# lhwright13/Hybrid-Classical-and-Reinforcement-Learning-Aircraft-Controllers

Hardware: AMD Instinct MI355X
Metric: env-steps/sec (whole node), rate-control task, batch 65536 per GPU (higher is better)
Workload: dtype f32 compute / f64 state

## Files before the change

### hybrid-classical-and-reinforcement-learning-aircraft-controllers_amd/_lib.py

```python
import ctypes as C
import os

_HERE = os.path.dirname(os.path.abspath(__file__))
LIB_PATH = os.environ.get("FDYN_LIB", os.path.join(_HERE, "csrc", "libfdyn_hip.so"))

FDYN_OK, FDYN_ERR_BAD_DT, FDYN_ERR_BAD_TYPES, FDYN_ERR_BAD_SIZE, FDYN_ERR_NULL = 0, -1, -2, -3, -4

_p = C.c_void_p
_i, _i64, _u64, _d, _f = C.c_int, C.c_int64, C.c_uint64, C.c_double, C.c_float

_SIXDOF = [_p, _p, _p, _p, _i, _i64, _d, _i, _p, _p]
_CASCADE = [_p, _p, _p, _p, _p, _i, _p, _p, _p, _i, _i64, _d, _i, _p, _p, _p]
_AGENT = [_i, _p, _p, _p, _p, _i, _p, _i, _p, _p, _i64, _d, _i, _p, _p]
_HYBRID = [_i, _p, _p, _p, _p, _p, _i, _p, _p, _p, _p, _i, _p, _p, _i, _p, _p, _p, _p, _p, _i64, _d, _p]
_ENV_RESET = [_p, _p, _p, _p, _p, _p, _p, _i, _u64, _p, _i64, _p]
_ENV_STEP = [_p, _p, _p, _p, _p, _i, _p, _p, _p, _p, _p, _p, _p, _p, _i, _u64, _i, _f, _p, _p, _p, _p, _p, _p, _p, _p, _p,
             _i, _i64, _p]
_ENV_RESET_DR = _ENV_RESET[:-1] + [_p, _p, _p]
_ENV_STEP_DR = _ENV_STEP[:-1] + [_p, _p, _p]

SIGNATURES = {
    "fdyn_abi_version": (_i, []),
    "fdyn_num_substeps": (_i, [_d, _d]),
    "fdyn_device_info": (_i, [C.POINTER(_i), C.POINTER(_i), C.c_char_p, _i]),
    "fdyn_event_capacity": (_i64, [_i64]),
    "fdyn_sixdof_step_f64": (_i, _SIXDOF), "fdyn_sixdof_step_mixed": (_i, _SIXDOF), "fdyn_sixdof_step_f32": (_i, _SIXDOF),
    "fdyn_derived_f64": (_i, [_p, _i64, _p, _p]), "fdyn_derived_f32": (_i, [_p, _i64, _p, _p]),
    "fdyn_pid_compute_batch": (_i, [_p, _i, _p, _p, _p, _f, _p, _i64, _p]),
    "fdyn_cascade_step_f64": (_i, _CASCADE), "fdyn_cascade_step_mixed": (_i, _CASCADE), "fdyn_cascade_step_f32": (_i, _CASCADE),
    "fdyn_rate_env_reset_f64": (_i, _ENV_RESET), "fdyn_rate_env_reset_mixed": (_i, _ENV_RESET),
    "fdyn_rate_env_reset_f32": (_i, _ENV_RESET),
    "fdyn_rate_env_step_f64": (_i, _ENV_STEP), "fdyn_rate_env_step_mixed": (_i, _ENV_STEP),
    "fdyn_rate_env_step_f32": (_i, _ENV_STEP),
    "fdyn_rate_env_reset_dr_f64": (_i, _ENV_RESET_DR), "fdyn_rate_env_reset_dr_mixed": (_i, _ENV_RESET_DR),
    "fdyn_rate_env_reset_dr_f32": (_i, _ENV_RESET_DR),
    "fdyn_rate_env_step_dr_f64": (_i, _ENV_STEP_DR), "fdyn_rate_env_step_dr_mixed": (_i, _ENV_STEP_DR),
    "fdyn_rate_env_step_dr_f32": (_i, _ENV_STEP_DR),
    "fdyn_lstm_cell_fwd": (_i, [_p, _i, _p, _p, _p, _p, _p, _i64, _i, _p]),
    "fdyn_lstm_cell_bwd": (_i, [_p, _i, _p, _p, _p, _p, _p, _p, _i64, _i, _p]),
    "fdyn_lstm_seq_fwd": (_i, [_p, _i, _p, _p, _p, _p, _p, _p, _i64, _p, _p, _i64, _i64, _i, _p]),
    "fdyn_lstm_seq_bwd": (_i, [_p, _i, _p, _p, _p, _p, _p, _i64, _p, _p, _p, _p, _i64, _i, _p]),
    "fdyn_lstm_seq_bwd_bsum": (_i, [_p, _i, _p, _p, _p, _p, _p, _i64, _p, _p, _p, _p, _p, _i64, _i64, _i, _p]),
    "fdyn_lstm_seq_bwd_pre": (_i, [_p, _i, _p, _i64, _p, _p, _p, _p, _p, _i64, _p, _p, _p, _p, _p, _i64, _i64, _i, _p]),
    "fdyn_lstm_cell0_fwd": (_i, [_p, _i, _p, _p, _i64, _i, _p]),
    "fdyn_lstm_cell0_bwd": (_i, [_p, _i, _p, _p, _p, _i64, _i64, _i, _p]),
    "fdyn_colsum_partials": (_i, [_p, _i64, _i, _p, _p, _p]),
    "fdyn_episode_flags": (_i, [_p, _p, _p, _p, _p, _i64, _p]),
    "fdyn_policy_trunks": (_i, [_p, _p, _p, _p, _p, _p, _p, _p, _i64, _p]),
    "fdyn_policy_trunks_heads": (_i, [_p] * 11 + [_u64, _p, _i, _p, _p, _p, _i64, _p]),
    "fdyn_agent_step_f64": (_i, _AGENT), "fdyn_agent_step_mixed": (_i, _AGENT), "fdyn_agent_step_f32": (_i, _AGENT),
    "fdyn_hybrid_step_f64": (_i, _HYBRID), "fdyn_hybrid_step_mixed": (_i, _HYBRID), "fdyn_hybrid_step_f32": (_i, _HYBRID),
    "fdyn_colsum_ws_floats": (_i64, [_i64, _i, _i64, _i]),
# ... 91 lines not shown
```

### hybrid-classical-and-reinforcement-learning-aircraft-controllers_amd/csrc/fdyn_kernels.hip

```cpp
#include <hip/hip_runtime.h>
#include <stdint.h>
#include <math.h>
#include <string.h>
#include <stdlib.h>
#include "fdyn_core.hpp"
#include "../../include/fdyn.h"

using namespace fdyn;

#define FD_BLOCK 256
#define FD_MAX_TYPES 8
#define FD_WAVE 64

template <typename T>
__device__ __forceinline__ void stage(T* dst, const T* __restrict__ src, int n)
{
    for (int i = threadIdx.x; i < n; i += blockDim.x) dst[i] = src[i];
}

template <bool FAST>
__device__ __forceinline__ void stage_params(double* s_params, const double* __restrict__ params, int n_types)
{
    for (int i = threadIdx.x; i < n_types * FD_NP_USED; i += blockDim.x) {
        const int t = i / FD_NP_USED, k = i - t * FD_NP_USED;
// ... 19 lines not shown
    w.d = int(threadIdx.x) < n_types * NDL ? params[t * FD_NP + Params<double>::derive_source(threadIdx.x - t * NDL)] : 1.0;
    return w;
}
template <bool FAST>
__device__ __forceinline__ void stage_params_finish(double* s_params, const StagedParamWords& w, int n_types)
{
    const int i0 = threadIdx.x, i1 = FD_BLOCK + threadIdx.x;
    const int t0 = i0 / FD_NP_USED, t1 = i1 / FD_NP_USED;
    if (i0 < n_types * FD_NP_USED) s_params[t0 * FD_NP_STAGED + (i0 - t0 * FD_NP_USED)] = w.v0;
    if (i1 < n_types * FD_NP_USED) s_params[t1 * FD_NP_STAGED + (i1 - t1 * FD_NP_USED)] = w.v1;
    constexpr int NDL = Params<double>::FD_ND_LANES;
    if (int(threadIdx.x) < n_types * NDL) {
        const int t = threadIdx.x / NDL;
        Params<double>::derive_lane_from<FAST>(threadIdx.x - t * NDL, w.d, s_params + t * FD_NP_STAGED);
    }
}

template <typename G>
__device__ __forceinline__ void stage_cascade_consts(G* s_consts, const double* __restrict__ consts)
{
    for (int k = threadIdx.x; k < FD_NC; k += blockDim.x) s_consts[k] = G(consts[k]);
    if (threadIdx.x < 2) {
        const double bank = consts[threadIdx.x == 0 ? FD_C_WP_MAX_BANK_RAD : FD_C_LOS_MAX_BANK_RAD];
        s_consts[FD_CD_WP_INV_G_TAN_BANK + threadIdx.x] = G(1.0 / (9.81 * ::tan(bank)));
    }
}

struct LaneMap { int64_t i, wave_first; int lane; bool on; };
__device__ __forceinline__ LaneMap lane_map(int64_t n)
{
// ... 537 lines not shown
    x[6] = rec[FD_R_ROLL]; x[7] = rec[FD_R_PITCH]; x[8] = rec[FD_R_YAW];
    x[9] = rec[FD_R_P]; x[10] = rec[FD_R_Q]; x[11] = rec[FD_R_R];
#pragma unroll
    for (int k = 0; k < 3; ++k) { e.cmd[k] = E(0); e.prev_err[k] = E(0); e.sign_changes[k] = E(0); e.prev_action[k] = E(0); }
#pragma unroll
    for (int k = 0; k < 4; ++k) e.sched[k] = E(0);
    e.prev_action[3] = E(0.5);
    if (cmd_type == FD_CMD_STEP) {
        e.cmd[0] = E(rec[FD_R_CMD0]); e.cmd[1] = E(rec[FD_R_CMD1]); e.cmd[2] = E(rec[FD_R_CMD2]);
    } else if (cmd_type == FD_CMD_RAMP || cmd_type == FD_CMD_SINE) {
        e.sched[0] = E(rec[FD_R_CMD0]); e.sched[1] = E(rec[FD_R_CMD1]); e.sched[2] = E(rec[FD_R_CMD2]); e.sched[3] = E(rec[FD_R_CMD3]);
    }
    e.settle_timer = E(0); e.is_settled = E(0); e.time = E(0); e.ep_return = E(0);
}

template <typename G>
__device__ __forceinline__ void load_env_consts(const double* __restrict__ EC, EnvConsts<G>& ec)
{
    ec.dt = G(EC[FD_EC_DT]);
    ec.max_steps = int(EC[FD_EC_MAX_STEPS]);
    ec.cmd_type = int(EC[FD_EC_CMD_TYPE]);
    ec.scale = G(EC[FD_EC_DIFFICULTY_SCALE]);
    ec.mr0 = G(EC[FD_EC_MAX_RATE_P]); ec.mr1 = G(EC[FD_EC_MAX_RATE_Q]); ec.mr2 = G(EC[FD_EC_MAX_RATE_R]);
    const double r = EC[FD_EC_DT] / EC[FD_EC_DT_PHYSICS];
    const long ns = long(r);
    ec.n_sub = ns < 1 ? 1 : int(ns);
    const double dts = EC[FD_EC_DT];
    int k = 0;
    if (dts >= 1.0e-3) { double t = 0.0; while (t < 0.2 && k < 256) { t += dts; ++k; } }
    else k = int(0.2 / dts) + 1;
    ec.settle_steps = k;
}

template <typename G>
__device__ __forceinline__ void fetch_reset_record(const double* __restrict__ pool, int pool_depth, uint64_t seed,
                                                   int64_t i, int32_t episode, const EnvConsts<G>& ec, G (&rec)[FD_NR])
{
    if (pool) {
        const double* r = pool + (i * pool_depth + (episode % pool_depth)) * FD_NR;
#pragma unroll
        for (int k = 0; k < FD_NR; ++k) rec[k] = G(r[k]);
    } else {
        device_reset_record<G>(seed, uint32_t(i), uint32_t(episode), ec, rec);
    }
}

__device__ __forceinline__ void store_obs_tile(float* tile , const float (&o)[FD_OBS_DIM], int lane,
                                               float* __restrict__ obs_out, int64_t wave_first, int64_t n)
{
    int64_t valid = n - wave_first;
    valid = valid < 0 ? 0 : (valid < FD_WAVE ? valid : FD_WAVE);
    float* dst = obs_out + wave_first * FD_OBS_DIM;
    static_assert(FD_OBS_DIM == 18 && FD_WAVE == 64, "the full-wave path below moves 64 x 18 floats as 288 float4");
    if (valid == FD_WAVE && (reinterpret_cast<uintptr_t>(dst) & 15) == 0) {
        float2* row = reinterpret_cast<float2*>(tile + lane * FD_OBS_DIM);
#pragma unroll
// ... 152 lines not shown
extern "C" int fdyn_debug_read_counts(unsigned* out, int count, int clear)
{
    int rc = int(hipMemcpyFromSymbol(out, HIP_SYMBOL(fdyn_dbg_cnt), sizeof(unsigned) * size_t(count)));
    if (clear && rc == 0) {
        void* p = nullptr;
        rc = int(hipGetSymbolAddress(&p, HIP_SYMBOL(fdyn_dbg_cnt)));
        if (rc == 0) rc = int(hipMemset(p, 0, sizeof(unsigned) * 4096 * 8));
    }
    return rc;
}
#else
#define FD_STAMP(K)
#define FD_STAMP_REAL(K)
#endif

template <typename S, typename T, bool OCC2, typename... DRA>
__global__ void __launch_bounds__(FD_BLOCK, OCC2 ? 2 : 1)
rate_env_step_kernel(S* __restrict__ xs, typename EnvOf<S, T>::type* __restrict__ es, int32_t* __restrict__ eis,
                     const uint8_t* __restrict__ type, const double* __restrict__ params, int n_types,
                     const double* __restrict__ EC,
                     const float* __restrict__ actions ,
                     float* __restrict__ pid_state , const float* __restrict__ pid_cfg ,
                     const double* __restrict__ casc_consts , float* __restrict__ actions_out,
                     const S* __restrict__ rw_delta ,
                     const double* __restrict__ pool, int pool_depth, uint64_t seed, int auto_reset, float residual_scale,
                     float* __restrict__ obs_out , float* __restrict__ reward_f32, S* __restrict__ reward_full,
                     uint8_t* __restrict__ terminated, uint8_t* __restrict__ truncated,
                     int32_t* __restrict__ ev_count, int32_t* __restrict__ ev_count_next, int32_t* __restrict__ ev_int,
                     float* __restrict__ ev_flt, int ev_cap, int64_t n, DRA... dra)
{
    constexpr bool DR = sizeof...(DRA) != 0;
    S* dr = nullptr;
    const double* drc = nullptr;
    if constexpr (DR) dr_unpack(dr, drc, dra...);
    __shared__ double s_params[FD_MAX_TYPES * FD_NP_STAGED];
    __shared__ __attribute__((aligned(16))) float s_tile[FD_BLOCK / FD_WAVE][FD_WAVE * (FD_OBS_DIM + 1)];
    __shared__ float s_pid_cfg[3 * FD_NPC];
    __shared__ S s_consts[FD_NC];
    FD_STAMP(0)
    FD_STAMP_REAL(7)
    const LaneMap lm = lane_map(n);
    const int64_t i = lm.i;
    const int lane = lm.lane, wave = threadIdx.x / FD_WAVE;
    const bool active = lm.on;
    EnvConsts<S> ec;
    load_env_consts<S>(EC, ec);
    const bool uses_sched = ec.cmd_type == FD_CMD_RAMP || ec.cmd_type == FD_CMD_SINE;
    const bool residual_mode = actions != nullptr && residual_scale > 0.0f && pid_state != nullptr;
    const bool pid_mode = actions == nullptr || residual_mode;

    using E = typename EnvOf<S, T>::type;
    S x[FD_NX];
    EnvState<E> e;
    int32_t step = 0, episode = 0;
    int ty = 0;
    float4 av = make_float4(0.0f, 0.0f, 0.0f, 0.0f);
    S rec_pre[FD_NR];
    S wair[3] = { S(0), S(0), S(0) }, dsc[5] = { S(1), S(1), S(1), S(1), S(1) };
    const bool pre_drawn = !OCC2 && pool == nullptr && auto_reset != 0;
    constexpr bool EARLY_PARAMS = sizeof(T) == 4;
    StagedParamWords spw = { 0.0, 0.0, 1.0 };
    if constexpr (EARLY_PARAMS) spw = stage_params_early(params, n_types);
    if (active) {
        episode = eis[FD_EI_EPISODE * n + i];
#pragma unroll
        for (int k = 3; k < FD_NX; ++k) x[k] = xs[k * n + i];
        if (actions) av = reinterpret_cast<const float4*>(actions)[i];
        ty = lane_type(type, i, n_types);
#pragma unroll
        for (int k = 0; k < 3; ++k) x[k] = xs[k * n + i];
        step = eis[FD_EI_STEP * n + i];
        env_load<E>(e, es, n, i, uses_sched);
        if (pre_drawn) device_reset_record<S>(seed, uint32_t(i), uint32_t(episode), ec, rec_pre);
        if constexpr (DR) {
#pragma unroll
            for (int k = 0; k < 3; ++k) wair[k] = dr[(FD_DR_WIND_N + k) * n + i] + dr[(FD_DR_GUST_N + k) * n + i];
#pragma unroll
            for (int k = 0; k < 5; ++k) dsc[k] = dr[(FD_DR_MASS_S + k) * n + i];
        }
    }
    if constexpr (EARLY_PARAMS) stage_params_finish<true>(s_params, spw, n_types);
    else stage_params<false>(s_params, params, n_types);
    if (pid_mode) {
        stage(s_pid_cfg, pid_cfg, 3 * FD_NPC);
        for (int k = threadIdx.x; k < FD_NC; k += blockDim.x) s_consts[k] = S(casc_consts[k]);
    }
    __syncthreads();

    if (ev_count_next && blockIdx.x == 0 && threadIdx.x < FD_EV_SHARDS) ev_count_next[threadIdx.x] = 0;

    float o[FD_OBS_DIM];
#pragma unroll
    for (int k = 0; k < FD_OBS_DIM; ++k) o[k] = 0.0f;
    bool done = false, term = false;
    S reward = S(0);

// ... 119 lines not shown
        if (reward_f32) reward_f32[i] = float(reward);
        if (reward_full) reward_full[i] = reward;
        terminated[i] = term ? 1 : 0;
        truncated[i] = trunc ? 1 : 0;
    }

    FD_STAMP(3)
    const unsigned long long done_mask = __ballot(done);
    const bool compact = done_mask != 0ull && ev_count != nullptr;
    int base = 0, prefix = 0;
    const int shard = int(blockIdx.x) & (FD_EV_SHARDS - 1), cap_s = ev_cap / FD_EV_SHARDS;
    if (compact) {
        const int n_done = __popcll(done_mask);
        prefix = __builtin_amdgcn_mbcnt_hi(uint32_t(done_mask >> 32), __builtin_amdgcn_mbcnt_lo(uint32_t(done_mask), 0u));
        const int leader = __ffsll((long long)done_mask) - 1;
        if (lane == leader) base = atomicAdd(ev_count + shard, n_done);
    }
    float o_term[FD_OBS_DIM];
#pragma unroll
    for (int k = 0; k < FD_OBS_DIM; ++k) o_term[k] = o[k];
    const float ret_term = done ? float(e.ep_return) : 0.0f;
    const int32_t len_term = step;

    if (active) {
        if (done && auto_reset) {
            S rec[FD_NR];
            if (pre_drawn) {
#pragma unroll
                for (int k = 0; k < FD_NR; ++k) rec[k] = rec_pre[k];
            } else {
                fetch_reset_record<S>(pool, pool_depth, seed, i, episode, ec, rec);
// ... 5 lines not shown
            using A0 = typename GlueOf<S, T>::type;
            A0 xa[FD_NX];
#pragma unroll
            for (int k = 0; k < FD_NX; ++k) xa[k] = A0(x[k]);
            A0 airspeed, altitude;
            airspeed_altitude<A0>(xa, airspeed, altitude);
            if constexpr (DR) airspeed = air_speed<A0, S>(x, wair);
            env_observation<S, A0, E>(x, e, airspeed, altitude, o);
            if (pid_mode) for (int k = 0; k < 3 * FD_NPS; ++k) pid_state[k * n + i] = 0.0f;
        }
#pragma unroll
        for (int k = 0; k < FD_NX; ++k) xs[k * n + i] = x[k];
        env_store<E>(e, es, n, i, uses_sched);
        eis[FD_EI_STEP * n + i] = step;
        eis[FD_EI_EPISODE * n + i] = episode;
    }
    if (compact) {
        const int leader = __ffsll((long long)done_mask) - 1;
        base = __shfl(base, leader, FD_WAVE);
        const int local = base + prefix;
        if (done && local < cap_s) {
            const int slot = shard * cap_s + local;
            ev_int[slot * FD_EV_NI + FD_EV_ENV] = int32_t(i);
            ev_int[slot * FD_EV_NI + FD_EV_LENGTH] = len_term;
            ev_int[slot * FD_EV_NI + FD_EV_TERMINATED] = term ? 1 : 0;
            ev_flt[slot * FD_EV_NF] = ret_term;
#pragma unroll
            for (int k = 0; k < FD_OBS_DIM; ++k) ev_flt[slot * FD_EV_NF + 1 + k] = o_term[k];
        }
    }
    FD_STAMP(4)
    store_obs_tile(s_tile[wave], o, lane, obs_out, lm.wave_first, n);
    FD_STAMP(5)
#ifdef FD_PHASE_STAMPS
    asm volatile("s_waitcnt vmcnt(0)" ::: "memory");
#endif
    FD_STAMP_REAL(6)
}

static int g_simds = 0;
static int simd_count()
{
    if (!g_simds) {
        int dev = 0; hipDeviceProp_t p;
        g_simds = (hipGetDevice(&dev) == hipSuccess && hipGetDeviceProperties(&p, dev) == hipSuccess) ? p.multiProcessorCount * 4 : 1024;
    }
    return g_simds;
}

template <typename K, typename... A>
static int launch(K kernel, int64_t n, void* stream, A... args)
{
// ... 20 lines not shown
    int32_t* ev_count_next, int32_t* ev_int, float* ev_flt, int ev_cap, int64_t n
#define FD_ENV_STEP_ARGS                                                                                     \
    x, e, ei, type, params, n_types, env_consts, actions, pid_state, pid_cfg, casc_consts, actions_out, rw_delta, pool, \
    pool_depth, seed, auto_reset, residual_scale, obs_out, reward_f32, reward_full, terminated, truncated, ev_count, \
    ev_count_next, ev_int, ev_flt, ev_cap, n

template <typename S, typename E, typename... DRA>
static int env_reset(FD_ENV_RESET_PARAMS(S, E), void* stream, DRA... dra)
{
    if ((... || !dra)) return FDYN_ERR_NULL;
    FD_CHECK_COMMON(n, 1)
    if (pool && pool_depth < 1) return FDYN_ERR_BAD_SIZE;
    return launch(rate_env_reset_kernel<S, E, DRA...>, n, stream, FD_ENV_RESET_ARGS, dra...);
}

template <typename S, typename E, typename T, typename... DRA>
static int env_step(FD_ENV_STEP_PARAMS(S, E), void* stream, DRA... dra)
{
    if ((... || !dra)) return FDYN_ERR_NULL;
    FD_CHECK_COMMON(n, n_types)
    if (pool && pool_depth < 1) return FDYN_ERR_BAD_SIZE;
    if ((!actions || residual_scale > 0.0f) && !(pid_state && pid_cfg && casc_consts)) return FDYN_ERR_NULL;
    if (!obs_out || !terminated || !truncated || !env_consts) return FDYN_ERR_NULL;
    if (ev_count && (!ev_int || !ev_flt)) return FDYN_ERR_NULL;
    if (ev_count && (ev_cap < FD_EV_SHARDS || ev_cap % FD_EV_SHARDS != 0)) return FDYN_ERR_BAD_SIZE;
    constexpr bool FP32 = sizeof(T) == 4;
    const bool occ2 = FP32 && n > int64_t(simd_count()) * FD_WAVE;
    return launch(occ2 ? rate_env_step_kernel<S, T, FP32, DRA...> : rate_env_step_kernel<S, T, false, DRA...>, n, stream,
                  FD_ENV_STEP_ARGS, dra...);
}

extern "C" {

int fdyn_abi_version(void) { return FDYN_ABI_VERSION; }

int fdyn_num_substeps(double dt, double dt_physics)
{
    const double r = dt / dt_physics;
    const long n = long(r);
    return n < 1 ? 1 : int(n);
}

int64_t fdyn_event_capacity(int64_t n)
// ... 94 lines not shown
                      consts, cmd, wps, n_wp, actions, learned, throttle_src, prev_action, obs_out, rate_cmd_out, surf_out, \
                      reached_total, n, S(dt));                                                              \
    }
FD_DEFINE_HYBRID(fdyn_hybrid_step_f64, double, double)
FD_DEFINE_HYBRID(fdyn_hybrid_step_mixed, double, float)
FD_DEFINE_HYBRID(fdyn_hybrid_step_f32, float, float)

FD_DEFINE_CASCADE(fdyn_cascade_step_f64, double, double)
FD_DEFINE_CASCADE(fdyn_cascade_step_mixed, double, float)
FD_DEFINE_CASCADE(fdyn_cascade_step_f32, float, float)

#define FD_DEFINE_ENV(SUFFIX, S, E, T)                                                                       \
    int fdyn_rate_env_reset_##SUFFIX(FD_ENV_RESET_PARAMS(S, E), void* stream)                                \
    { return env_reset<S, E>(FD_ENV_RESET_ARGS, stream); }                                                   \
    int fdyn_rate_env_step_##SUFFIX(FD_ENV_STEP_PARAMS(S, E), void* stream)                                  \
    { return env_step<S, E, T>(FD_ENV_STEP_ARGS, stream); }
FD_DEFINE_ENV(f64, double, double, double)
FD_DEFINE_ENV(mixed, double, float, float)
FD_DEFINE_ENV(f32, float, float, float)

#define FD_DEFINE_ENV_DR(SUFFIX, S, E, T)                                                                    \
    int fdyn_rate_env_reset_dr_##SUFFIX(FD_ENV_RESET_PARAMS(S, E), S* dr, const double* dr_consts, void* stream) \
    { return env_reset<S, E>(FD_ENV_RESET_ARGS, stream, dr, dr_consts); }                                    \
    int fdyn_rate_env_step_dr_##SUFFIX(FD_ENV_STEP_PARAMS(S, E), S* dr, const double* dr_consts, void* stream) \
    { return env_step<S, E, T>(FD_ENV_STEP_ARGS, stream, dr, dr_consts); }
FD_DEFINE_ENV_DR(f64, double, double, double)
FD_DEFINE_ENV_DR(mixed, double, float, float)
FD_DEFINE_ENV_DR(f32, float, float, float)

}
```

### hybrid-classical-and-reinforcement-learning-aircraft-controllers_amd/rate_env.py

```python
from typing import Optional, Sequence

import numpy as np
import torch

from . import _lib, layout as L
from .config import cascade_consts, pid_table
from .params import param_table
from .samplers import COMMAND_TYPE, EpisodeStreams, env_consts, presample_reset_pool


class GpuRateVecEnv:
    def __init__(self, num_envs: int, difficulty: str = "medium", episode_length: float = 10.0, dt: float = 0.02,
                 command_type: str = "step", seed: Optional[int] = None, precision: str = "mixed",
                 sampling: str = "device", pool_depth: int = 8, types: Sequence = ("rc_plane",),
                 type_index: Optional[np.ndarray] = None, event_capacity: Optional[int] = None,
                 numpy_io: bool = False, device=None, residual_scale: float = 0.0, sensor_noise: Optional[dict] = None,
                 disturbances=None):
        self.lib = _lib.load()
        self.device = device or _lib.require_gpu()
        self.num_envs = self.n = int(num_envs)
        self.precision, self.dtype = precision, _lib.state_dtype(precision)
        self.difficulty, self.episode_length, self.dt, self.command_type = difficulty, episode_length, dt, command_type
        self.seed_value = 0 if seed is None else int(seed)
        self.numpy_io = numpy_io
# ... 31 lines not shown
        self.pool, self.pool_depth, self._streams = None, 0, None
        if sampling == "parity":
            seeds = [None if seed is None else seed + i for i in range(n)]
            self.pool_depth = int(pool_depth)
            self.pool = torch.as_tensor(presample_reset_pool(seeds, pool_depth, difficulty, command_type), device=dev)
            if command_type == "random":
                self._streams = [EpisodeStreams(difficulty, command_type, s) for s in seeds]
        elif sampling != "device":
            raise ValueError("sampling must be 'parity' or 'device'")
        self.sensor = None
        if sensor_noise is not None:
            from .sensors import ObservationNoise
            self.sensor = ObservationNoise(sensor_noise, n, dev)
            self._done_mask = torch.zeros(n, dtype=torch.uint8, device=dev)
        self._reset_fn = getattr(self.lib, f"fdyn_rate_env_reset_{precision}")
        self._step_fn = getattr(self.lib, f"fdyn_rate_env_step_{precision}")
        self._pending = None
        self.dr, self.dr_consts, self.disturbances = None, None, None
        if disturbances is not None:
            self.set_disturbances(disturbances)

    def set_disturbances(self, d):
        from .disturbances import Disturbances, as_disturbances, neutral_rows
        d = as_disturbances(d)
        if d is None:
            d = Disturbances()
        self.disturbances = d
        blk = torch.as_tensor(d.block(), device=self.device)
        if self.dr_consts is None:
            self.dr_consts = blk
            self.dr = torch.as_tensor(neutral_rows(self.n), device=self.device).to(self.dtype).contiguous()
            self._reset_fn = getattr(self.lib, f"fdyn_rate_env_reset_dr_{self.precision}")
            self._step_fn = getattr(self.lib, f"fdyn_rate_env_step_dr_{self.precision}")
        else:
            self.dr_consts.copy_(blk)
        return d

    def _dr_args(self):
        return () if self.dr is None else (_lib.ptr(self.dr), _lib.ptr(self.dr_consts))

    def reset(self, mask: Optional[torch.Tensor] = None):
        m = None if mask is None else mask.to(torch.uint8).contiguous()
        rc = self._reset_fn(_lib.ptr(self.x), _lib.ptr(self.e), _lib.ptr(self.ei), _lib.ptr(self.pid_state),
                            _lib.ptr(m), _lib.ptr(self.env_consts), _lib.ptr(self.pool), self.pool_depth,
                            self.seed_value, _lib.ptr(self.obs), self.n, *self._dr_args(), _lib.current_stream())
        _lib.check(rc, "RateControlEnv.reset")
        if self.sensor is not None:
            if m is None:
                self.sensor.reset()
                self.sensor.apply(self.obs)
            else:
                keep, keep_bias, mb = self.obs.clone(), self.sensor.gyro_bias.clone(), m.bool()
                self.sensor.apply(self.obs, m)
                self.obs.copy_(torch.where(mb[:, None], self.obs, keep))
                self.sensor.gyro_bias.copy_(torch.where(mb[None, :], self.sensor.gyro_bias, keep_bias))
        return self._out(self.obs)

    def step_device(self, actions: Optional[torch.Tensor], auto_reset: bool = True, rw_delta=None):
        if actions is not None:
            actions = actions.to(device=self.device, dtype=torch.float32).contiguous()
            assert actions.shape == (self.n, L.FD_ACT_DIM)
        if rw_delta is not None:
            assert rw_delta.shape == (3, self.n) and rw_delta.dtype == self.dtype and rw_delta.device == self.x.device
        acts_out = self.actions_taken if (actions is None or self.residual_scale > 0.0) else None
        cur, nxt = self._ev_counts[self._ev_slot], self._ev_counts[1 - self._ev_slot]
        self._ev_cur, self._ev_slot = cur, 1 - self._ev_slot
        rc = self._step_fn(_lib.ptr(self.x), _lib.ptr(self.e), _lib.ptr(self.ei), _lib.ptr(self.type_index),
                           _lib.ptr(self.params), self.n_types, _lib.ptr(self.env_consts), _lib.ptr(actions),
                           _lib.ptr(self.pid_state), _lib.ptr(self.pid_cfg), _lib.ptr(self.casc_consts),
                           _lib.ptr(acts_out), _lib.ptr(rw_delta), _lib.ptr(self.pool), self.pool_depth,
                           self.seed_value, int(auto_reset), self.residual_scale, _lib.ptr(self.obs), _lib.ptr(self.rewards),
                           _lib.ptr(self.rewards_full), _lib.ptr(self.terminated), _lib.ptr(self.truncated),
                           cur.data_ptr(), nxt.data_ptr(), _lib.ptr(self.ev_int), _lib.ptr(self.ev_flt), self.ev_cap,
                           self.n, *self._dr_args(), _lib.current_stream())
        _lib.check(rc, "RateControlEnv.step")
        if self.sensor is not None:
            mask = None
            if auto_reset:
                torch.bitwise_or(self.terminated, self.truncated, out=self._done_mask)
                mask = self._done_mask
            self.sensor.apply(self.obs, mask)
        return self.obs, self.rewards, self.terminated, self.truncated

    def mark_episode_starts(self):
        self.terminated.fill_(1)
        self.truncated.zero_()

    def step(self, actions, auto_reset: bool = True):
        if isinstance(actions, np.ndarray):
# ... 117 lines not shown
```

### include/fdyn.h

```cpp
#ifndef FDYN_H
#define FDYN_H

#include <stdint.h>
#include "fdyn_layout.h"

#ifdef __cplusplus
extern "C" {
#endif

#define FDYN_ABI_VERSION 3

#define FDYN_OK 0
#define FDYN_ERR_BAD_DT (-1)
#define FDYN_ERR_BAD_TYPES (-2)
#define FDYN_ERR_BAD_SIZE (-3)
#define FDYN_ERR_NULL (-4)

int fdyn_abi_version(void);
int fdyn_num_substeps(double dt, double dt_physics);
int fdyn_device_info(int* cu_count , int* wave_size , char* arch , int arch_len);
int64_t fdyn_event_capacity(int64_t n);

int fdyn_sixdof_step_f64(double* x, const double* u, const uint8_t* type, const double* params, int n_types,
                         int64_t n, double dt, int n_sub, double* derived_out, void* stream);
// ... 75 lines not shown
                                const double* casc_consts, float* actions_out, const double* rw_delta, const double* pool,
                                int pool_depth, uint64_t seed, int auto_reset, float residual_scale, float* obs_out,
                                float* reward_f32, double* reward_full, uint8_t* terminated, uint8_t* truncated, int32_t* ev_count,
                                int32_t* ev_count_next, int32_t* ev_int, float* ev_flt, int ev_cap, int64_t n, double* dr,
                                const double* dr_consts, void* stream);
int fdyn_rate_env_reset_dr_f32(float* x, float* e, int32_t* ei, float* pid_state, const uint8_t* mask, const double* env_consts,
                               const double* pool, int pool_depth, uint64_t seed, float* obs_out, int64_t n, float* dr,
                               const double* dr_consts, void* stream);
int fdyn_rate_env_step_dr_f32(float* x, float* e, int32_t* ei, const uint8_t* type, const double* params, int n_types,
                              const double* env_consts, const float* actions, float* pid_state, const float* pid_cfg,
                              const double* casc_consts, float* actions_out, const float* rw_delta, const double* pool,
                              int pool_depth, uint64_t seed, int auto_reset, float residual_scale, float* obs_out,
                              float* reward_f32, float* reward_full, uint8_t* terminated, uint8_t* truncated, int32_t* ev_count,
                              int32_t* ev_count_next, int32_t* ev_int, float* ev_flt, int ev_cap, int64_t n, float* dr,
                              const double* dr_consts, void* stream);

int fdyn_lstm_cell_fwd(const void* gates, int gates_bf16, const float* c_prev, float* h_f32, void* h_lp, float* c_out,
                       void* act_out, int64_t B, int H, void* stream);
int fdyn_lstm_cell_bwd(const void* act, int bf16, const float* c_prev, const float* c_new, const void* dh,
                       const float* dc_next, void* dgates, float* dc_prev, int64_t B, int H, void* stream);
int fdyn_lstm_seq_fwd(const void* gates, int gates_bf16, const float* c_prev, const float* keep, void* h_lp, float* c_out,
                      void* act_out, void* h_next, int64_t next_stride, const float* keep_next, const void* bias,
                      int64_t group_rows, int64_t B, int H, void* stream);
int fdyn_lstm_seq_bwd(const void* act, int bf16, const float* c_prev, const float* keep, const float* c_new, const void* dh,
                      const void* dh2, int64_t dh2_stride, const float* dh2_keep, const float* dc_next, void* dgates,
                      float* dc_prev, int64_t B, int H, void* stream);
int fdyn_lstm_seq_bwd_bsum(const void* act, int bf16, const float* c_prev, const float* keep, const float* c_new, const void* dh,
                           const void* dh2, int64_t dh2_stride, const float* dh2_keep, const float* dc_next, void* dgates,
                           float* dc_prev, float* bias_ws, int64_t rows_per_block, int64_t B, int H, void* stream);
int fdyn_lstm_seq_bwd_pre(const void* gates, int bf16, const void* bias, int64_t group_rows, const float* c_prev, const float* keep,
// ... 75 lines not shown
```

### include/fdyn_layout.h

```cpp
#ifndef FDYN_LAYOUT_H
#define FDYN_LAYOUT_H

enum {
    FD_X_N = 0, FD_X_E, FD_X_D,
    FD_X_U, FD_X_V, FD_X_W,
    FD_X_ROLL, FD_X_PITCH, FD_X_YAW,
    FD_X_P, FD_X_Q, FD_X_R,
    FD_NX = 12
};

enum { FD_U_ELEVATOR = 0, FD_U_AILERON, FD_U_RUDDER, FD_U_THROTTLE, FD_NU = 4 };

enum { FD_D_AIRSPEED = 0, FD_D_ALTITUDE, FD_D_GROUND_SPEED, FD_D_HEADING, FD_ND = 4 };

enum {
    FD_P_MASS = 0, FD_P_IXX, FD_P_IYY, FD_P_IZZ,
    FD_P_WING_AREA, FD_P_WING_SPAN, FD_P_CHORD,
    FD_P_CL_0, FD_P_CL_ALPHA, FD_P_CD_0, FD_P_CD_ALPHA2,
    FD_P_CL_ELEVATOR, FD_P_CM_ELEVATOR, FD_P_CY_RUDDER, FD_P_CN_RUDDER, FD_P_CL_AILERON,
    FD_P_CM_ALPHA, FD_P_CN_BETA, FD_P_CL_BETA,
    FD_P_DAMPING_ROLL, FD_P_DAMPING_PITCH, FD_P_DAMPING_YAW,
    FD_P_MAX_THRUST, FD_P_AIR_DENSITY, FD_P_GRAVITY,
    FD_P_MIN_AIRSPEED_AERO, FD_P_MIN_U_VELOCITY,
    FD_P_MAX_ELEVATOR_RAD, FD_P_MAX_AILERON_RAD, FD_P_MAX_RUDDER_RAD,
// ... 52 lines not shown
    FD_E_TIME,
    FD_E_SCHED0, FD_E_SCHED1, FD_E_SCHED2,
    FD_E_SCHED3,
    FD_E_EP_RETURN,
    FD_NE = 21
};
enum { FD_EI_STEP = 0, FD_EI_EPISODE, FD_NEI = 2 };

enum {
    FD_EC_DT = 0, FD_EC_DT_PHYSICS, FD_EC_MAX_STEPS, FD_EC_CMD_TYPE, FD_EC_DIFFICULTY_SCALE,
    FD_EC_MAX_RATE_P, FD_EC_MAX_RATE_Q, FD_EC_MAX_RATE_R,
    FD_NEC = 8
};

enum {
    FD_R_AIRSPEED = 0, FD_R_ALTITUDE, FD_R_ROLL, FD_R_PITCH, FD_R_YAW, FD_R_P, FD_R_Q, FD_R_R,
    FD_R_CMD0, FD_R_CMD1, FD_R_CMD2,
    FD_R_CMD3,
    FD_NR = 12
};

enum { FD_EV_ENV = 0, FD_EV_LENGTH, FD_EV_TERMINATED, FD_EV_NI = 3 };
#define FD_EV_NF (1 + FD_OBS_DIM)
enum { FD_EV_SHARDS = 64 };

enum {
    FD_DR_WIND_N = 0, FD_DR_WIND_E, FD_DR_WIND_D,
    FD_DR_GUST_N, FD_DR_GUST_E, FD_DR_GUST_D,
    FD_DR_GUST_A, FD_DR_GUST_B,
    FD_DR_MASS_S, FD_DR_IXX_S, FD_DR_IYY_S, FD_DR_IZZ_S, FD_DR_RHO_S,
// ... 46 lines not shown
```

Before: 1.735 billion.

## Precompute staged parameter and env-constant image once, reuse across step launches

Adds a one-block kernel that derives the per-type staged parameter blocks and integer env constants (max_steps, cmd_type, n_sub, settle_steps) into a cached device image. The step kernel then copies that image into shared memory instead of re-deriving the parameters in every block on every launch. The image is rebuilt only when the tensor versions or pointers change. The change also moves the event-compaction writes inside the active branch and adds asm barriers to steer register allocation, which could alter scheduling.

```diff
diff --git a/hybrid-classical-and-reinforcement-learning-aircraft-controllers_amd/_lib.py b/hybrid-classical-and-reinforcement-learning-aircraft-controllers_amd/_lib.py
--- a/hybrid-classical-and-reinforcement-learning-aircraft-controllers_amd/_lib.py
+++ b/hybrid-classical-and-reinforcement-learning-aircraft-controllers_amd/_lib.py
@@ -18,6 +18,8 @@
              _i, _i64, _p]
 _ENV_RESET_DR = _ENV_RESET[:-1] + [_p, _p, _p]
 _ENV_STEP_DR = _ENV_STEP[:-1] + [_p, _p, _p]
+_ENV_STEP_IMG = _ENV_STEP[:-1] + [_p, _p]
+_ENV_STEP_DR_IMG = _ENV_STEP_DR[:-1] + [_p, _p]
 
 SIGNATURES = {
     "fdyn_abi_version": (_i, []),
@@ -36,6 +38,11 @@
     "fdyn_rate_env_reset_dr_f32": (_i, _ENV_RESET_DR),
     "fdyn_rate_env_step_dr_f64": (_i, _ENV_STEP_DR), "fdyn_rate_env_step_dr_mixed": (_i, _ENV_STEP_DR),
     "fdyn_rate_env_step_dr_f32": (_i, _ENV_STEP_DR),
+    "fdyn_rate_env_image": (_i, [_p, _i, _p, _i, _p, _p]),
+    "fdyn_rate_env_step_img_f64": (_i, _ENV_STEP_IMG), "fdyn_rate_env_step_img_mixed": (_i, _ENV_STEP_IMG),
+    "fdyn_rate_env_step_img_f32": (_i, _ENV_STEP_IMG),
+    "fdyn_rate_env_step_dr_img_f64": (_i, _ENV_STEP_DR_IMG), "fdyn_rate_env_step_dr_img_mixed": (_i, _ENV_STEP_DR_IMG),
+    "fdyn_rate_env_step_dr_img_f32": (_i, _ENV_STEP_DR_IMG),
     "fdyn_lstm_cell_fwd": (_i, [_p, _i, _p, _p, _p, _p, _p, _i64, _i, _p]),
     "fdyn_lstm_cell_bwd": (_i, [_p, _i, _p, _p, _p, _p, _p, _p, _i64, _i, _p]),
     "fdyn_lstm_seq_fwd": (_i, [_p, _i, _p, _p, _p, _p, _p, _p, _i64, _p, _p, _i64, _i64, _i, _p]),
diff --git a/hybrid-classical-and-reinforcement-learning-aircraft-controllers_amd/csrc/fdyn_kernels.hip b/hybrid-classical-and-reinforcement-learning-aircraft-controllers_amd/csrc/fdyn_kernels.hip
--- a/hybrid-classical-and-reinforcement-learning-aircraft-controllers_amd/csrc/fdyn_kernels.hip
+++ b/hybrid-classical-and-reinforcement-learning-aircraft-controllers_amd/csrc/fdyn_kernels.hip
@@ -57,6 +57,22 @@
         const int t = threadIdx.x / NDL;
         Params<double>::derive_lane_from<FAST>(threadIdx.x - t * NDL, w.d, s_params + t * FD_NP_STAGED);
     }
+}
+
+__device__ __forceinline__ StagedParamWords stage_image_early(const double* __restrict__ staged, int n_types)
+{
+    StagedParamWords w;
+    const int i0 = threadIdx.x, i1 = FD_BLOCK + threadIdx.x;
+    w.v0 = i0 < n_types * FD_NP_STAGED ? staged[i0] : 0.0;
+    w.v1 = i1 < n_types * FD_NP_STAGED ? staged[i1] : 0.0;
+    w.d = 1.0;
+    return w;
+}
+__device__ __forceinline__ void stage_image_finish(double* s_params, const StagedParamWords& w, int n_types)
+{
+    const int i0 = threadIdx.x, i1 = FD_BLOCK + threadIdx.x;
+    if (i0 < n_types * FD_NP_STAGED) s_params[i0] = w.v0;
+    if (i1 < n_types * FD_NP_STAGED) s_params[i1] = w.v1;
 }
 
 template <typename G>
@@ -624,14 +640,21 @@
     e.settle_timer = E(0); e.is_settled = E(0); e.time = E(0); e.ep_return = E(0);
 }
 
-template <typename G>
+template <typename G, bool PREP = false>
 __device__ __forceinline__ void load_env_consts(const double* __restrict__ EC, EnvConsts<G>& ec)
 {
     ec.dt = G(EC[FD_EC_DT]);
-    ec.max_steps = int(EC[FD_EC_MAX_STEPS]);
-    ec.cmd_type = int(EC[FD_EC_CMD_TYPE]);
+    if constexpr (!PREP) {
+        ec.max_steps = int(EC[FD_EC_MAX_STEPS]);
+        ec.cmd_type = int(EC[FD_EC_CMD_TYPE]);
+    }
     ec.scale = G(EC[FD_EC_DIFFICULTY_SCALE]);
     ec.mr0 = G(EC[FD_EC_MAX_RATE_P]); ec.mr1 = G(EC[FD_EC_MAX_RATE_Q]); ec.mr2 = G(EC[FD_EC_MAX_RATE_R]);
+    if constexpr (PREP) {
+        const int32_t* __restrict__ ic = reinterpret_cast<const int32_t*>(EC + FD_ECD_INTS);
+        ec.max_steps = ic[0]; ec.cmd_type = ic[1]; ec.n_sub = ic[2]; ec.settle_steps = ic[3];
+        return;
+    }
     const double r = EC[FD_EC_DT] / EC[FD_EC_DT_PHYSICS];
     const long ns = long(r);
     ec.n_sub = ns < 1 ? 1 : int(ns);
@@ -650,6 +673,8 @@
         const double* r = pool + (i * pool_depth + (episode % pool_depth)) * FD_NR;
 #pragma unroll
         for (int k = 0; k < FD_NR; ++k) rec[k] = G(r[k]);
+#pragma unroll
+        for (int k = 0; k < FD_NR; ++k) asm volatile("" : "+v"(rec[k]));
     } else {
         device_reset_record<G>(seed, uint32_t(i), uint32_t(episode), ec, rec);
     }
@@ -832,7 +857,7 @@
 #define FD_STAMP_REAL(K)
 #endif
 
-template <typename S, typename T, bool OCC2, typename... DRA>
+template <typename S, typename T, bool OCC2, bool PREP, typename... DRA>
 __global__ void __launch_bounds__(FD_BLOCK, OCC2 ? 2 : 1)
 rate_env_step_kernel(S* __restrict__ xs, typename EnvOf<S, T>::type* __restrict__ es, int32_t* __restrict__ eis,
                      const uint8_t* __restrict__ type, const double* __restrict__ params, int n_types,
@@ -862,7 +887,7 @@
     const int lane = lm.lane, wave = threadIdx.x / FD_WAVE;
     const bool active = lm.on;
     EnvConsts<S> ec;
-    load_env_consts<S>(EC, ec);
+    load_env_consts<S, PREP>(EC, ec);
     const bool uses_sched = ec.cmd_type == FD_CMD_RAMP || ec.cmd_type == FD_CMD_SINE;
     const bool residual_mode = actions != nullptr && residual_scale > 0.0f && pid_state != nullptr;
     const bool pid_mode = actions == nullptr || residual_mode;
@@ -878,7 +903,7 @@
     const bool pre_drawn = !OCC2 && pool == nullptr && auto_reset != 0;
     constexpr bool EARLY_PARAMS = sizeof(T) == 4;
     StagedParamWords spw = { 0.0, 0.0, 1.0 };
-    if constexpr (EARLY_PARAMS) spw = stage_params_early(params, n_types);
+    if constexpr (EARLY_PARAMS) spw = PREP ? stage_image_early(params, n_types) : stage_params_early(params, n_types);
     if (active) {
         episode = eis[FD_EI_EPISODE * n + i];
 #pragma unroll
@@ -897,7 +922,10 @@
             for (int k = 0; k < 5; ++k) dsc[k] = dr[(FD_DR_MASS_S + k) * n + i];
         }
     }
-    if constexpr (EARLY_PARAMS) stage_params_finish<true>(s_params, spw, n_types);
+    if constexpr (PREP) {
+        if constexpr (EARLY_PARAMS) stage_image_finish(s_params, spw, n_types);
+        else stage(s_params, params, n_types * FD_NP_STAGED);
+    } else if constexpr (EARLY_PARAMS) stage_params_finish<true>(s_params, spw, n_types);
     else stage_params<false>(s_params, params, n_types);
     if (pid_mode) {
         stage(s_pid_cfg, pid_cfg, 3 * FD_NPC);
@@ -1047,7 +1075,11 @@
         const int n_done = __popcll(done_mask);
         prefix = __builtin_amdgcn_mbcnt_hi(uint32_t(done_mask >> 32), __builtin_amdgcn_mbcnt_lo(uint32_t(done_mask), 0u));
         const int leader = __ffsll((long long)done_mask) - 1;
-        if (lane == leader) base = atomicAdd(ev_count + shard, n_done);
+        if (lane == leader) {
+            int cnt = shard;
+            asm volatile("" : "+v"(cnt));
+            base = atomicAdd(ev_count + cnt, n_done);
+        }
     }
     float o_term[FD_OBS_DIM];
 #pragma unroll
@@ -1083,19 +1115,20 @@
         env_store<E>(e, es, n, i, uses_sched);
         eis[FD_EI_STEP * n + i] = step;
         eis[FD_EI_EPISODE * n + i] = episode;
-    }
-    if (compact) {
-        const int leader = __ffsll((long long)done_mask) - 1;
-        base = __shfl(base, leader, FD_WAVE);
-        const int local = base + prefix;
-        if (done && local < cap_s) {
-            const int slot = shard * cap_s + local;
-            ev_int[slot * FD_EV_NI + FD_EV_ENV] = int32_t(i);
-            ev_int[slot * FD_EV_NI + FD_EV_LENGTH] = len_term;
-            ev_int[slot * FD_EV_NI + FD_EV_TERMINATED] = term ? 1 : 0;
-            ev_flt[slot * FD_EV_NF] = ret_term;
-#pragma unroll
-            for (int k = 0; k < FD_OBS_DIM; ++k) ev_flt[slot * FD_EV_NF + 1 + k] = o_term[k];
+        if (compact) {
+            asm volatile("" : "+v"(base) : : "memory");
+            const int leader = __ffsll((long long)done_mask) - 1;
+            base = __shfl(base, leader, FD_WAVE);
+            const int local = base + prefix;
+            if (done && local < cap_s) {
+                const int slot = shard * cap_s + local;
+                ev_int[slot * FD_EV_NI + FD_EV_ENV] = int32_t(i);
+                ev_int[slot * FD_EV_NI + FD_EV_LENGTH] = len_term;
+                ev_int[slot * FD_EV_NI + FD_EV_TERMINATED] = term ? 1 : 0;
+                ev_flt[slot * FD_EV_NF] = ret_term;
+#pragma unroll
+                for (int k = 0; k < FD_OBS_DIM; ++k) ev_flt[slot * FD_EV_NF + 1 + k] = o_term[k];
+            }
         }
     }
     FD_STAMP(4)
@@ -1105,6 +1138,31 @@
     asm volatile("s_waitcnt vmcnt(0)" ::: "memory");
 #endif
     FD_STAMP_REAL(6)
+}
+
+static_assert(FD_NIMG == FD_IMG_PARAMS + FD_MAX_TYPES * FD_NP_STAGED && FD_ECD_INTS + 2 <= FD_IMG_PARAMS, "fdyn_layout.h: image sections");
+template <bool FAST>
+__global__ void __launch_bounds__(FD_BLOCK)
+rate_env_image_kernel(const double* __restrict__ params, int n_types, const double* __restrict__ EC, double* __restrict__ image)
+{
+    double* blocks = image + FD_IMG_PARAMS;
+    for (int i = threadIdx.x; i < FD_MAX_TYPES * FD_NP_STAGED; i += blockDim.x) {
+        const int t = i / FD_NP_STAGED, k = i - t * FD_NP_STAGED;
+        blocks[i] = (t < n_types && k < FD_NP_USED) ? params[t * FD_NP + k] : 0.0;
+    }
+    for (int k = threadIdx.x; k < FD_IMG_PARAMS; k += blockDim.x) if (k < FD_ECD_INTS || k >= FD_ECD_INTS + 2) image[FD_IMG_EC + k] = k < FD_NEC ? EC[k] : 0.0;
+    __syncthreads();
+    constexpr int NDL = Params<double>::FD_ND_LANES;
+    if (int(threadIdx.x) < n_types * NDL) {
+        const int t = threadIdx.x / NDL;
+        Params<double>::derive_lane<FAST>(threadIdx.x - t * NDL, params + t * FD_NP, blocks + t * FD_NP_STAGED);
+    }
+    if (threadIdx.x == FD_BLOCK - 1) {
+        EnvConsts<double> ec;
+        load_env_consts<double>(EC, ec);
+        int32_t* ic = reinterpret_cast<int32_t*>(image + FD_IMG_EC + FD_ECD_INTS);
+        ic[0] = ec.max_steps; ic[1] = ec.cmd_type; ic[2] = ec.n_sub; ic[3] = ec.settle_steps;
+    }
 }
 
 static int g_simds = 0;
@@ -1155,7 +1213,7 @@
     return launch(rate_env_reset_kernel<S, E, DRA...>, n, stream, FD_ENV_RESET_ARGS, dra...);
 }
 
-template <typename S, typename E, typename T, typename... DRA>
+template <typename S, typename E, typename T, bool PREP, typename... DRA>
 static int env_step(FD_ENV_STEP_PARAMS(S, E), void* stream, DRA... dra)
 {
     if ((... || !dra)) return FDYN_ERR_NULL;
@@ -1167,7 +1225,7 @@
     if (ev_count && (ev_cap < FD_EV_SHARDS || ev_cap % FD_EV_SHARDS != 0)) return FDYN_ERR_BAD_SIZE;
     constexpr bool FP32 = sizeof(T) == 4;
     const bool occ2 = FP32 && n > int64_t(simd_count()) * FD_WAVE;
-    return launch(occ2 ? rate_env_step_kernel<S, T, FP32, DRA...> : rate_env_step_kernel<S, T, false, DRA...>, n, stream,
+    return launch(occ2 ? rate_env_step_kernel<S, T, FP32, PREP, DRA...> : rate_env_step_kernel<S, T, false, PREP, DRA...>, n, stream,
                   FD_ENV_STEP_ARGS, dra...);
 }
 
@@ -1292,7 +1350,7 @@
     int fdyn_rate_env_reset_##SUFFIX(FD_ENV_RESET_PARAMS(S, E), void* stream)                                \
     { return env_reset<S, E>(FD_ENV_RESET_ARGS, stream); }                                                   \
     int fdyn_rate_env_step_##SUFFIX(FD_ENV_STEP_PARAMS(S, E), void* stream)                                  \
-    { return env_step<S, E, T>(FD_ENV_STEP_ARGS, stream); }
+    { return env_step<S, E, T, false>(FD_ENV_STEP_ARGS, stream); }
 FD_DEFINE_ENV(f64, double, double, double)
 FD_DEFINE_ENV(mixed, double, float, float)
 FD_DEFINE_ENV(f32, float, float, float)
@@ -1301,9 +1359,34 @@
     int fdyn_rate_env_reset_dr_##SUFFIX(FD_ENV_RESET_PARAMS(S, E), S* dr, const double* dr_consts, void* stream) \
     { return env_reset<S, E>(FD_ENV_RESET_ARGS, stream, dr, dr_consts); }                                    \
     int fdyn_rate_env_step_dr_##SUFFIX(FD_ENV_STEP_PARAMS(S, E), S* dr, const double* dr_consts, void* stream) \
-    { return env_step<S, E, T>(FD_ENV_STEP_ARGS, stream, dr, dr_consts); }
+    { return env_step<S, E, T, false>(FD_ENV_STEP_ARGS, stream, dr, dr_consts); }
 FD_DEFINE_ENV_DR(f64, double, double, double)
 FD_DEFINE_ENV_DR(mixed, double, float, float)
 FD_DEFINE_ENV_DR(f32, float, float, float)
 
-}
+int fdyn_rate_env_image(const double* params, int n_types, const double* env_consts, int fp32_eval, double* image, void* stream)
+{
+    if (n_types < 1 || n_types > FD_MAX_TYPES) return FDYN_ERR_BAD_TYPES;
+    if (!params || !env_consts || !image) return FDYN_ERR_NULL;
+    return launch(fp32_eval ? rate_env_image_kernel<true> : rate_env_image_kernel<false>, FD_BLOCK, stream, params, n_types,
+                  env_consts, image);
+}
+#define FD_DEFINE_ENV_IMG(SUFFIX, S, E, T)                                                                   \
+    int fdyn_rate_env_step_img_##SUFFIX(FD_ENV_STEP_PARAMS(S, E), const double* image, void* stream)         \
+    {                                                                                                        \
+        if (!image) return FDYN_ERR_NULL;                                                                    \
+        params = image + FD_IMG_PARAMS; env_consts = image + FD_IMG_EC;                                      \
+        return env_step<S, E, T, true>(FD_ENV_STEP_ARGS, stream);                                            \
+    }                                                                                                        \
+    int fdyn_rate_env_step_dr_img_##SUFFIX(FD_ENV_STEP_PARAMS(S, E), S* dr, const double* dr_consts, const double* image, \
+                                           void* stream)                                                     \
+    {                                                                                                        \
+        if (!image) return FDYN_ERR_NULL;                                                                    \
+        params = image + FD_IMG_PARAMS; env_consts = image + FD_IMG_EC;                                      \
+        return env_step<S, E, T, true>(FD_ENV_STEP_ARGS, stream, dr, dr_consts);                             \
+    }
+FD_DEFINE_ENV_IMG(f64, double, double, double)
+FD_DEFINE_ENV_IMG(mixed, double, float, float)
+FD_DEFINE_ENV_IMG(f32, float, float, float)
+
+}
diff --git a/hybrid-classical-and-reinforcement-learning-aircraft-controllers_amd/rate_env.py b/hybrid-classical-and-reinforcement-learning-aircraft-controllers_amd/rate_env.py
--- a/hybrid-classical-and-reinforcement-learning-aircraft-controllers_amd/rate_env.py
+++ b/hybrid-classical-and-reinforcement-learning-aircraft-controllers_amd/rate_env.py
@@ -7,6 +7,33 @@
 from .config import cascade_consts, pid_table
 from .params import param_table
 from .samplers import COMMAND_TYPE, EpisodeStreams, env_consts, presample_reset_pool
+
+
+class LaunchImage:
+
+    def __init__(self, precision, fill):
+        self.fp32_eval = precision != "f64"
+        self._fill = fill
+        self.image = None
+        self._key = None
+        self.fills = 0
+
+    @staticmethod
+    def key(params, n_types, env_consts):
+        return (params.data_ptr(), params._version, int(n_types), env_consts.data_ptr(), env_consts._version)
+
+    def ensure(self, params, n_types, env_consts):
+        k = self.key(params, n_types, env_consts)
+        if k != self._key:
+            if self.image is None:
+                self.image = torch.zeros(L.FD_NIMG, dtype=torch.float64, device=params.device)
+            self._fill(params, n_types, env_consts, self.fp32_eval, self.image)
+            self._key = self.key(params, n_types, env_consts)
+            self.fills += 1
+        return self.image
+
+    def invalidate(self):
+        self._key = None
 
 
 class GpuRateVecEnv:
@@ -69,7 +96,9 @@
             self.sensor = ObservationNoise(sensor_noise, n, dev)
             self._done_mask = torch.zeros(n, dtype=torch.uint8, device=dev)
         self._reset_fn = getattr(self.lib, f"fdyn_rate_env_reset_{precision}")
-        self._step_fn = getattr(self.lib, f"fdyn_rate_env_step_{precision}")
+        self._step_fn = getattr(self.lib, f"fdyn_rate_env_step_img_{precision}")
+        self._image = LaunchImage(precision, self._fill_image)
+        self.launch_image()
         self._pending = None
         self.dr, self.dr_consts, self.disturbances = None, None, None
         if disturbances is not None:
@@ -86,10 +115,20 @@
             self.dr_consts = blk
             self.dr = torch.as_tensor(neutral_rows(self.n), device=self.device).to(self.dtype).contiguous()
             self._reset_fn = getattr(self.lib, f"fdyn_rate_env_reset_dr_{self.precision}")
-            self._step_fn = getattr(self.lib, f"fdyn_rate_env_step_dr_{self.precision}")
+            self._step_fn = getattr(self.lib, f"fdyn_rate_env_step_dr_img_{self.precision}")
         else:
             self.dr_consts.copy_(blk)
         return d
+
+    def _fill_image(self, params, n_types, env_consts, fp32_eval, image):
+        assert params.dtype == torch.float64 and env_consts.dtype == torch.float64
+        assert params.shape == (n_types, L.FD_NP) and env_consts.numel() == L.FD_NEC
+        rc = self.lib.fdyn_rate_env_image(_lib.ptr(params), n_types, _lib.ptr(env_consts), int(fp32_eval), _lib.ptr(image),
+                                          _lib.current_stream())
+        _lib.check(rc, "RateControlEnv launch image")
+
+    def launch_image(self):
+        return self._image.ensure(self.params, self.n_types, self.env_consts)
 
     def _dr_args(self):
         return () if self.dr is None else (_lib.ptr(self.dr), _lib.ptr(self.dr_consts))
@@ -120,6 +159,7 @@
         acts_out = self.actions_taken if (actions is None or self.residual_scale > 0.0) else None
         cur, nxt = self._ev_counts[self._ev_slot], self._ev_counts[1 - self._ev_slot]
         self._ev_cur, self._ev_slot = cur, 1 - self._ev_slot
+        image = self.launch_image()
         rc = self._step_fn(_lib.ptr(self.x), _lib.ptr(self.e), _lib.ptr(self.ei), _lib.ptr(self.type_index),
                            _lib.ptr(self.params), self.n_types, _lib.ptr(self.env_consts), _lib.ptr(actions),
                            _lib.ptr(self.pid_state), _lib.ptr(self.pid_cfg), _lib.ptr(self.casc_consts),
@@ -127,7 +167,7 @@
                            self.seed_value, int(auto_reset), self.residual_scale, _lib.ptr(self.obs), _lib.ptr(self.rewards),
                            _lib.ptr(self.rewards_full), _lib.ptr(self.terminated), _lib.ptr(self.truncated),
                            cur.data_ptr(), nxt.data_ptr(), _lib.ptr(self.ev_int), _lib.ptr(self.ev_flt), self.ev_cap,
-                           self.n, *self._dr_args(), _lib.current_stream())
+                           self.n, *self._dr_args(), _lib.ptr(image), _lib.current_stream())
         _lib.check(rc, "RateControlEnv.step")
         if self.sensor is not None:
             mask = None
diff --git a/include/fdyn.h b/include/fdyn.h
--- a/include/fdyn.h
+++ b/include/fdyn.h
@@ -113,6 +113,44 @@
                               float* reward_f32, float* reward_full, uint8_t* terminated, uint8_t* truncated, int32_t* ev_count,
                               int32_t* ev_count_next, int32_t* ev_int, float* ev_flt, int ev_cap, int64_t n, float* dr,
                               const double* dr_consts, void* stream);
+
+int fdyn_rate_env_image(const double* params, int n_types, const double* env_consts, int fp32_eval, double* image, void* stream);
+int fdyn_rate_env_step_img_f64(double* x, double* e, int32_t* ei, const uint8_t* type, const double* params, int n_types,
+    const double* env_consts, const float* actions, float* pid_state, const float* pid_cfg, const double* casc_consts,
+    float* actions_out, const double* rw_delta, const double* pool, int pool_depth, uint64_t seed, int auto_reset,
+    float residual_scale, float* obs_out, float* reward_f32, double* reward_full, uint8_t* terminated, uint8_t* truncated,
+    int32_t* ev_count, int32_t* ev_count_next, int32_t* ev_int, float* ev_flt, int ev_cap, int64_t n, const double* image,
+    void* stream);
+int fdyn_rate_env_step_dr_img_f64(double* x, double* e, int32_t* ei, const uint8_t* type, const double* params, int n_types,
+    const double* env_consts, const float* actions, float* pid_state, const float* pid_cfg, const double* casc_consts,
+    float* actions_out, const double* rw_delta, const double* pool, int pool_depth, uint64_t seed, int auto_reset,
+    float residual_scale, float* obs_out, float* reward_f32, double* reward_full, uint8_t* terminated, uint8_t* truncated,
+    int32_t* ev_count, int32_t* ev_count_next, int32_t* ev_int, float* ev_flt, int ev_cap, int64_t n, double* dr,
+    const double* dr_consts, const double* image, void* stream);
+int fdyn_rate_env_step_img_mixed(double* x, float* e, int32_t* ei, const uint8_t* type, const double* params, int n_types,
+    const double* env_consts, const float* actions, float* pid_state, const float* pid_cfg, const double* casc_consts,
+    float* actions_out, const double* rw_delta, const double* pool, int pool_depth, uint64_t seed, int auto_reset,
+    float residual_scale, float* obs_out, float* reward_f32, double* reward_full, uint8_t* terminated, uint8_t* truncated,
+    int32_t* ev_count, int32_t* ev_count_next, int32_t* ev_int, float* ev_flt, int ev_cap, int64_t n, const double* image,
+    void* stream);
+int fdyn_rate_env_step_dr_img_mixed(double* x, float* e, int32_t* ei, const uint8_t* type, const double* params, int n_types,
+    const double* env_consts, const float* actions, float* pid_state, const float* pid_cfg, const double* casc_consts,
+    float* actions_out, const double* rw_delta, const double* pool, int pool_depth, uint64_t seed, int auto_reset,
+    float residual_scale, float* obs_out, float* reward_f32, double* reward_full, uint8_t* terminated, uint8_t* truncated,
+    int32_t* ev_count, int32_t* ev_count_next, int32_t* ev_int, float* ev_flt, int ev_cap, int64_t n, double* dr,
+    const double* dr_consts, const double* image, void* stream);
+int fdyn_rate_env_step_img_f32(float* x, float* e, int32_t* ei, const uint8_t* type, const double* params, int n_types,
+    const double* env_consts, const float* actions, float* pid_state, const float* pid_cfg, const double* casc_consts,
+    float* actions_out, const float* rw_delta, const double* pool, int pool_depth, uint64_t seed, int auto_reset,
+    float residual_scale, float* obs_out, float* reward_f32, float* reward_full, uint8_t* terminated, uint8_t* truncated,
+    int32_t* ev_count, int32_t* ev_count_next, int32_t* ev_int, float* ev_flt, int ev_cap, int64_t n, const double* image,
+    void* stream);
+int fdyn_rate_env_step_dr_img_f32(float* x, float* e, int32_t* ei, const uint8_t* type, const double* params, int n_types,
+    const double* env_consts, const float* actions, float* pid_state, const float* pid_cfg, const double* casc_consts,
+    float* actions_out, const float* rw_delta, const double* pool, int pool_depth, uint64_t seed, int auto_reset,
+    float residual_scale, float* obs_out, float* reward_f32, float* reward_full, uint8_t* terminated, uint8_t* truncated,
+    int32_t* ev_count, int32_t* ev_count_next, int32_t* ev_int, float* ev_flt, int ev_cap, int64_t n, float* dr,
+    const double* dr_consts, const double* image, void* stream);
 
 int fdyn_lstm_cell_fwd(const void* gates, int gates_bf16, const float* c_prev, float* h_f32, void* h_lp, float* c_out,
                        void* act_out, int64_t B, int H, void* stream);
diff --git a/include/fdyn_layout.h b/include/fdyn_layout.h
--- a/include/fdyn_layout.h
+++ b/include/fdyn_layout.h
@@ -90,6 +90,12 @@
 };
 
 enum {
+    FD_ECD_INTS = FD_NEC,
+    FD_IMG_EC = 0, FD_IMG_PARAMS = 16,
+    FD_NIMG = FD_IMG_PARAMS + 8 * FD_NP_STAGED
+};
+
+enum {
     FD_R_AIRSPEED = 0, FD_R_ALTITUDE, FD_R_ROLL, FD_R_PITCH, FD_R_YAW, FD_R_P, FD_R_Q, FD_R_R,
     FD_R_CMD0, FD_R_CMD1, FD_R_CMD2,
     FD_R_CMD3,
```

Result: faster. 1.789 billion (median of 6 runs) (+3.1%).
